# lboss75/vds

Measured on AMD Instinct MI355X. Metric: device-resident encode+repair GiB/s, k=16 m=4 64 MiB stripes, 1/2/4/8 GPU, higher is better.
Workload: dtype u16

## Files before the change

vds_amd/csrc/restore_syn.hpp:

```cpp
#pragma once

#include "ec_device.hpp"

namespace vds_ec {

constexpr int64_t kNoBound = 0x7FFFFFFFFFFFFFFFll;

template <int K, int N, int WV> struct RestorePrograms;

template <int K, int N, int WV>
struct SynShape {
  static constexpr int kWaves = WV;
  static constexpr int kThreads = 64 * WV;
  static constexpr int kM = N - K;
  static constexpr int kLoadPer = K / WV;
  using P = RestorePrograms<K, N, WV>;
  static constexpr int kSynRows = P::kSynRows;
  static constexpr int kCells = P::kIntRows / 16;
  static constexpr int kLdsBytes = N * 16 * 64 * 4;
  static constexpr int kWavesPerSimd = (160 * 1024 / kLdsBytes) * WV / 4;
  static constexpr bool kPrio = 160 * 1024 / kLdsBytes >= 2;
  static_assert(K % WV == 0 && kM <= WV, "survivor loads and erased slots must map onto waves");
  static_assert(kSynRows == 16 && kM == WV, "scatter recovery needs one whole syndrome per wave");
  static_assert(kCells == 2 || kCells == 4, "row split must be b128 / word-group aligned");
// ... 129 lines not shown
      if (first[c])
#pragma unroll
        for (int b = 0; b < 16; ++b) cells[16 * (c0 + c) + b] = 0u;
  }
}

template <int K, int N, int WV, int W>
__device__ __forceinline__ void syn_interp_gm(int wave, const SynLds &L, uint32_t (&cells)[16 * (K / WV)], Stamps &st) {
  static_assert((K == 16 && WV == 4) || (K == 32 && WV == 8),
                "the one-level interpolation is laid out for k = 16 and k = 32");
  using P = RestorePrograms<K, N, WV>;
  constexpr int kPairs = (K / 2) / WV;
  constexpr int kHalfCells = P::kHalfRows / 16;
  constexpr int kParts = WV / 2;
  constexpr bool kPrio = SynShape<K, N, WV>::kPrio;
  if constexpr (W < WV) {
    if (wave != W) return syn_interp_gm<K, N, WV, W + 1>(wave, L, cells, st);
    syn_prio<1, kPrio>();
    syn_gm_stage_a<W, kPairs>(L);
    syn_prio<0, kPrio>();
    st.mark(7);
    __syncthreads();
    st.mark(8);
    uint32_t half[P::kHalfRows];
    P::interpB(W, L, half);
    st.mark(9);
    __syncthreads();
    st.mark(10);
#pragma unroll
    for (int c = 0; c < kHalfCells; ++c) {
      uint32_t v[16];
#pragma unroll
      for (int b = 0; b < 16; ++b) v[b] = half[16 * c + b];
      syn_put_point(L, (K / 2) * (W / kParts) + kHalfCells * (W % kParts) + c, v);
    }
    st.mark(11);
    __syncthreads();
    st.mark(12);
    syn_gm_stage_c<K, W, K / WV>(L, cells);
    st.mark(13);
  }
}

template <int EP>
struct S1In {
  const SynLds &L;
  const Plane16 &own;
  __device__ __forceinline__ u32x4 operator()(int g) const {
    if ((g >> 2) == EP) return u32x4{own.p[4 * (g & 3)], own.p[4 * (g & 3) + 1], own.p[4 * (g & 3) + 2], own.p[4 * (g & 3) + 3]};
    return L(g);
  }
};

#ifndef VDS_GM2
#define VDS_GM2 1
#endif
#ifndef VDS_GM2_PRIO
#define VDS_GM2_PRIO 9
#endif
#ifndef VDS_HALF_PRIO
#define VDS_HALF_PRIO 1
#endif
template <int K, int N, int WV, int W, class Tail, class OwnP = void>
__device__ __forceinline__ void syn_interp_gm2(int wave, const SynLds &L, Stamps &st, Tail &&tail,
                                               const Plane16 *own = nullptr) {
  using P = RestorePrograms<K, N, WV>;
  constexpr bool kPrio = SynShape<K, N, WV>::kPrio;
  constexpr int H = K / 2, kWpf = WV / 4, kWpq = WV / 2;
  if constexpr (W < WV) {
    if (wave != W) return syn_interp_gm2<K, N, WV, W + 1, Tail &, OwnP>(wave, L, st, tail, own);
    uint32_t cells[16 * (K / WV)];
    uint32_t acc[64];
    auto cell = [&](int c) -> uint32_t(&)[16] { return *reinterpret_cast<uint32_t(*)[16]>(acc + 16 * c); };
    syn_prio<1, kPrio && (VDS_GM2_PRIO & 1)>();
    if constexpr (__is_same(OwnP, void))
      P::gm_s1_(W, L, acc);
    else
      P::gm_s1_(W, S1In<OwnP::kPoint[W]>{L, *own}, acc);
#pragma unroll
    for (int c = 0; c < 4; ++c) syn_put_point(L, 4 * W + c, cell(c));
    syn_prio<0, kPrio && (VDS_GM2_PRIO & 1)>();
    st.mark(7);
    __syncthreads();
    st.mark(8);
    syn_prio<1, kPrio && (VDS_GM2_PRIO & 2)>();
    P::gm_s2_(W, L, acc);
    constexpr int f = W / kWpf, c0 = 4 * (W % kWpf);
    if constexpr (kWpf > 1) {
      __syncthreads();
      constexpr int h = W % kWpf;
      static_assert(kWpf == 2 && K / 4 == 8, "plane-split S2 is laid out for k = 32");
#pragma unroll
      for (int c = 0; c < 8; ++c)
#pragma unroll
        for (int g = 0; g < 2; ++g)
          L.put(4 * (4 * c + f) + 2 * h + g,
                u32x4{acc[8 * c + 4 * g], acc[8 * c + 4 * g + 1], acc[8 * c + 4 * g + 2], acc[8 * c + 4 * g + 3]});
    } else {
#pragma unroll
      for (int c = 0; c < 4; ++c) syn_put_point(L, 4 * (c0 + c) + f, cell(c));
    }
    syn_prio<0, kPrio && (VDS_GM2_PRIO & 2)>();
    st.mark(9);
    __syncthreads();
    st.mark(10);
    syn_prio<1, kPrio && (VDS_GM2_PRIO & 4)>();
    P::gm_s3sum_(W, L, acc);
    constexpr int par = W / kWpq, i0 = 4 * (W % kWpq);
#pragma unroll
    for (int c = 0; c < 4; ++c) P::gm_twist(i0 + c, cell(c));
    syn_prio<0, kPrio && (VDS_GM2_PRIO & 4)>();
    __syncthreads();
#pragma unroll
    for (int c = 0; c < 4; ++c) syn_put_point(L, H * par + i0 + c, cell(c));
    st.mark(11);
    __syncthreads();
    st.mark(12);
    syn_prio<1, kPrio && (VDS_GM2_PRIO & 8)>();
    syn_gm_stage_c<K, W, K / WV>(L, cells);
    syn_prio<0, kPrio && (VDS_GM2_PRIO & 8)>();
    st.mark(13);
    tail(cells);
  }
}

#define VDS_RS_C(i) [c##i] "+v"(acc.p[i])
#define VDS_RS_A(i) [a##i] "v"(t.p[i])
#define VDS_RS_B(i) [b##i] "v"(t1.p[i])
#define VDS_RS_LIST(M) M(0), M(1), M(2), M(3), M(4), M(5), M(6), M(7), M(8), M(9), M(10), M(11), M(12), M(13), M(14), M(15)
#define VDS_RS_SEQ(M) M(0) M(1) M(2) M(3) M(4) M(5) M(6) M(7) M(8) M(9) M(10) M(11) M(12) M(13) M(14) M(15)
#define VDS_RS_XA(i) "v_xor_b32 %[c" #i "], %[c" #i "], %[a" #i "]\n"
#define VDS_RS_XB(i) "v_xor_b32 %[c" #i "], %[c" #i "], %[b" #i "]\n"
#define VDS_RS_X3(i) "v_bitop3_b32 %[c" #i "], %[c" #i "], %[a" #i "], %[b" #i "] bitop3:0x96\n"
__device__ __forceinline__ void rec_pair(Plane16 &acc, const Plane16 &t, const Plane16 &t1, uint32_t two) {
// ... 95 lines not shown
    return -1;
  }
  __device__ __forceinline__ u32x4 operator()(int idx) const {
    const int i = slot(idx >> 2), g = idx & 3;
    return u32x4{P[i].p[4 * g], P[i].p[4 * g + 1], P[i].p[4 * g + 2], P[i].p[4 * g + 3]};
  }
};
template <int WV, class FillP, bool REGS, int W>
__device__ __forceinline__ void syn_scatter_fill(int wave, const SynLds &L, const Plane16 (&Ps)[4]) {
  if constexpr (W < WV) {
    if (wave != W) return syn_scatter_fill<WV, FillP, REGS, W + 1>(wave, L, Ps);
#pragma unroll
    for (int q = 0; q < FillP::kParts; ++q) {
      uint32_t acc[16 * FillP::kPart];
      if constexpr (REGS)
        FillP::fill_part(q, W, FillRegIn<FillP, W>{Ps}, acc);
      else
        FillP::fill_part(q, W, L, acc);
#pragma unroll
      for (int m = 0; m < FillP::kPart; ++m)
        if (q * FillP::kPart + m < FillP::kFill)
          lds_xor_point(L, FillP::kPoint[q * FillP::kPart + m < FillP::kFill ? q * FillP::kPart + m : 0],
                        *reinterpret_cast<const Plane16 *>(acc + 16 * m));
    }
  }
}

template <class F, class = void>
struct FillOwn {
  static constexpr bool value = false;
};
template <class F>
struct FillOwn<F, decltype(void(F::kOwn))> {
  static constexpr bool value = F::kOwn;
};
template <class FillP, int W>
struct OwnIn {
  const SynLds &L;
  const Plane16 (&P)[4];
  __device__ __forceinline__ u32x4 operator()(int idx) const {
    const int i = FillRegIn<FillP, W>::slot(idx >> 2), g = idx & 3;
    if (i >= 0) return u32x4{P[i].p[4 * g], P[i].p[4 * g + 1], P[i].p[4 * g + 2], P[i].p[4 * g + 3]};
    return L(idx);
  }
};
template <int WV, class FillP, int W>
__device__ __forceinline__ void syn_own_fill(int wave, const SynLds &L, const Plane16 (&Ps)[4], Plane16 &own) {
  if constexpr (W < WV) {
    if (wave != W) return syn_own_fill<WV, FillP, W + 1>(wave, L, Ps, own);
    FillP::template own<W>(OwnIn<FillP, W>{L, Ps}, own.p);
  }
}

__device__ __forceinline__ u32x4 ld16_guard(const uint8_t *p, int64_t valid) {
  if (valid >= 16) return g_ld<4, u32x4>(p);
  u32x4 v = {0u, 0u, 0u, 0u};
  if (valid > 0) {
#pragma unroll
    for (int i = 0; i < 3; ++i)
      if (4 * i + 4 <= valid) v[i] = *(const gmem<uint32_t> *)(p + 4 * i);
    if (valid & 2) v[valid >> 2] = *(const gmem<uint16_t> *)(p + (valid & ~3));
  }
  return v;
}
__device__ __forceinline__ void st16_guard(uint8_t *p, u32x4 v, int64_t valid) {
  if (valid >= 16) {
    g_st<8>(p, v);
  } else if (valid > 0) {
#pragma unroll
    for (int i = 0; i < 3; ++i)
      if (4 * i + 4 <= valid) *(gmem<uint32_t> *)(p + 4 * i) = v[i];
    const int w = (int)(valid >> 2);
    const uint32_t x = v[w];
    for (int b = 0; b < (int)(valid & 3); ++b) ((gmem<uint8_t> *)p)[4 * w + b] = uint8_t(x >> (8 * b));
  }
}

struct NoFill {
  static constexpr int kFill = -1;
  static constexpr bool kScatter = false;
  static constexpr bool kSmall = false;
  static constexpr bool kPerm = false;
  static constexpr bool kMulti = false;
};
constexpr uint32_t kClsSyn = 0, kClsSmall1 = 1, kClsSmall2 = 2, kClsPerm = 3;
template <int K> struct MultiP {
  static constexpr int kFill = -1;
  static constexpr bool kScatter = false, kSmall = false, kPerm = false, kMulti = true;
};
template <class T> struct TypeTag {
  using type = T;
};
template <int K> struct PermSyn;
template <int K, int MS> struct SmallSyn;
#ifndef VDS_SYN_RT2
#define VDS_SYN_RT2 1
#endif
#ifndef VDS_BATCH_DUAL
#define VDS_BATCH_DUAL 1
#endif
#ifndef VDS_RT2_SPREAD
#define VDS_RT2_SPREAD 1
#endif
template <int K, int N, int WV, bool REGEN, bool BATCH, bool RT = false, class FillP = NoFill>
__device__ __forceinline__ void restore_syn_body(const SynRestoreArgs &a) {
  constexpr bool FILL = FillP::kFill >= 0;
  constexpr bool kScatter = FILL && FillP::kScatter;
  constexpr bool kOwn = FILL && FillOwn<FillP>::value;
  static_assert(!kOwn || (K == 16 && !REGEN && !BATCH && !RT), "the own-group fill is a k = 16 restore form");
  constexpr bool kSmall = FillP::kSmall;
  constexpr bool kPerm = FillP::kPerm;
  constexpr bool kMulti = FillP::kMulti;
  static_assert(!kMulti || (BATCH && !RT), "MULTI is a batch mode");
  static_assert(!kSmall || (BATCH && !RT && !FILL), "SMALL is a batch mode of its own");
  static_assert(!kPerm || (BATCH && REGEN && !RT && !FILL), "PERM is a batch regenerate mode of its own");
  using S = SynShape<K, N, WV>;
  using P = typename S::P;
  constexpr bool kPrio = S::kPrio;
  static_assert(!RT || BATCH, "RT is a batch mode");
  extern __shared__ __attribute__((aligned(16))) uint32_t lds[];
  const int lane = threadIdx.x & 63;
  const int wave = __builtin_amdgcn_readfirstlane(threadIdx.x >> 6);
  const BitMasks bm = bit_masks();
  if constexpr (!kPrio && VDS_HALF_PRIO)
    if (wave >= WV / 2) __builtin_amdgcn_s_setprio(1);
  SynLds L;
  L.base = (lds_char *)lds;
  L.lo = 16u * lane;
  L.hi = 16u * lane + 65536u;
  asm volatile("" : "+v"(L.hi));
  if constexpr (N * 16 > 128) {
    L.hi2 = 16u * lane + 131072u;
    asm volatile("" : "+v"(L.hi2));
  } else {
    L.hi2 = L.hi;
  }
  auto obj_of = [&](uint32_t t) -> uint32_t { return t / a.tiles_per_obj; };
  auto stripe0_of = [&](uint32_t t) -> uint64_t { return (uint64_t)(t % a.tiles_per_obj) * kTileStripes; };
  auto half_obj = [&](uint32_t t, int h) -> const SynBatchObj & { return a.objs[s_ld(&a.tiles[t].obj[h])]; };
  auto half_s0 = [&](uint32_t t, int h) -> uint64_t { return s_ld(&a.tiles[t].stripe0[h]); };

  u32x4 Q[S::kLoadPer][4];
  auto load = [&](uint32_t t) {
    if constexpr (BATCH) {
#pragma unroll
      for (int h = 0; h < 2; ++h) {
        const SynBatchObj &d = half_obj(t, h);
        const uint64_t st0 = half_s0(t, h);
        const int64_t valid = (int64_t)s_ld(&d.chunk_len) - (int64_t)(2 * st0);
        const uint8_t *src[S::kLoadPer];
#pragma unroll
        for (int s = 0; s < S::kLoadPer; ++s) src[s] = s_ld(&d.chunks[wave * S::kLoadPer + s]) + 2 * st0 + 16 * lane;
        if (valid >= 2 * (int64_t)kHalfStripes) {
#pragma unroll
          for (int s = 0; s < S::kLoadPer; ++s)
#pragma unroll
            for (int q = 0; q < 2; ++q) Q[s][2 * h + q] = g_ld<4, u32x4>(src[s] + 1024 * q);
        } else {
#pragma unroll
          for (int s = 0; s < S::kLoadPer; ++s)
#pragma unroll
            for (int q = 0; q < 2; ++q) Q[s][2 * h + q] = ld16_guard(src[s] + 1024 * q, valid - 16 * lane - 1024 * q);
        }
      }
    } else {
      const uint32_t ob = obj_of(t);
      const uint64_t st0 = stripe0_of(t);
#pragma unroll
      for (int s = 0; s < S::kLoadPer; ++s) {
        const uint8_t *src = a.chunks[wave * S::kLoadPer + s] + (uint64_t)ob * a.chunk_stride + 2 * st0 + 16 * lane;
#pragma unroll
        for (int q = 0; q < 4; ++q) Q[s][q] = g_ld<4, u32x4>(src + 1024 * q);
      }
    }
  };
  const TileRange tr = tile_range(a.total_tiles);
  Stamps st;
  st.init();
  auto prefetch = [&](uint32_t t) {
    if (t < tr.end && (VDS_DIAG_LOADS != 2 || t == tr.first)) {
      st.rt((t - tr.first) / tr.step);
      load(VDS_DIAG_LOADS == 1 ? tr.first : t);
    } else {
#pragma unroll
      for (int s = 0; s < S::kLoadPer; ++s)
#pragma unroll
        for (int q = 0; q < 4; ++q) Q[s][q] = u32x4{0u, 0u, 0u, 0u};
    }
  };
  constexpr bool kLateLoad = ((K == 32 || BATCH) && !REGEN) || RT;
  const uint32_t t_step = tr.step;
  prefetch(tr.first);
  if constexpr (!REGEN && !BATCH) {
    if (tr.first < tr.end) {
      const uint32_t t0 = tr.first;
      uint8_t *g0 = a.out + (uint64_t)(t0 / a.tiles_per_obj) * a.out_stride +
                    (uint64_t)(t0 % a.tiles_per_obj) * kTileStripes * (2 * K) + 16384u * wave + 16u * lane;
#pragma unroll
      for (int i = 0; i < 16; ++i) g_st<8>(g0 + 1024 * i, u32x4{0u, 0u, 0u, 0u});
    }
  }
  for (uint32_t tile = tr.first; tile < tr.end; tile += t_step) {
    const uint32_t o = BATCH ? 0u : obj_of(tile);
    const uint64_t stripe0 = BATCH ? 0u : stripe0_of(tile);
    const SynBatchPlan *pl = (BATCH && !RT) ? &a.plans[s_ld(&a.tiles[tile].plan)] : nullptr;
    auto erased_of = [&](int m) -> int { return (int)s_ld_u8(BATCH ? pl->erased : a.erased, m); };
    const uint32_t cls = kMulti ? s_ld(&pl->cls) : (kPerm ? kClsPerm : kClsSyn);
    const bool perm_tile = kPerm || (kMulti && REGEN && cls == kClsPerm);
    const int my_erased = RT ? K + wave : perm_tile ? K : (wave < S::kM ? erased_of(wave) : 0);
    constexpr bool kFillRegs = kScatter && VDS_FILL_REGS && K == 16;
    constexpr bool kKeepPs = RT || kFillRegs || kOwn;
    Plane16 own;
    static_assert(!kKeepPs || S::kLoadPer == 4, "four survivors per wave");
    Plane16 Ps[kKeepPs ? S::kLoadPer : 1];

    constexpr bool kRt2 = VDS_SYN_RT2 && RT && !REGEN && K == 32 && N >= K + 8;
    const bool rt2_tile = kRt2 && s_ld(&a.tiles[tile].mode) == 1u;
    constexpr bool kDual = VDS_BATCH_DUAL && BATCH && !RT && !FILL && !kSmall && !kPerm && K == 32;
    const bool dual_tile = kDual && s_ld(&a.tiles[tile].mode) == kTileDual;
    const SynBatchPlan *pl1 = kDual && dual_tile ? &a.plans[s_ld(&half_obj(tile, 1).plan)] : pl;
    syn_prio<1, kPrio>();
    uint64_t bor[2] = {0, 0};
    {
      if constexpr (kDual) {
        if (dual_tile) {
          static_assert(N % WV == 0, "dual tiles: whole slots per wave");
          const u32x4 z = {0u, 0u, 0u, 0u};
#pragma unroll
          for (int i = 0; i < N / WV; ++i)
#pragma unroll
            for (int g = 0; g < 4; ++g) L.put(4 * ((N / WV) * wave + i) + g, z);
          __syncthreads();
        }
      }
      if (wave < S::kM && (!RT || REGEN) && !FILL && (!perm_tile || wave == 0) && !(kDual && dual_tile)) {
        const u32x4 z = {0u, 0u, 0u, 0u};
#pragma unroll
        for (int g = 0; g < 4; ++g) L.put(4 * my_erased + g, z);
      }
      if constexpr (kScatter) {
        if (wave < FillP::kFill) {
          const u32x4 z = {0u, 0u, 0u, 0u};
#pragma unroll
          for (int g = 0; g < 4; ++g) L.put(4 * (int)FillP::kPoint[wave < FillP::kFill ? wave : 0] + g, z);
        }
      }
      if (rt2_tile) {
        const u32x4 z = {0u, 0u, 0u, 0u};
#pragma unroll
        for (int g = 0; g < 4; ++g) L.put(4 * (K + wave) + g, z);
      }
      if constexpr (RT && !REGEN) {
        bor[0] = s_ld(&half_obj(tile, 0).rt.borrowed);
        bor[1] = s_ld(&half_obj(tile, 1).rt.borrowed);
      }
#pragma unroll
      for (int s = 0; s < S::kLoadPer; ++s) {
        uint32_t W[16];
#pragma unroll
        for (int q = 0; q < 4; ++q)
#pragma unroll
          for (int d = 0; d < 4; ++d) W[4 * q + d] = Q[s][q][d];
        transpose16x2(W, bm);
        uint32_t Pl[16];
#pragma unroll
        for (int b = 0; b < 16; ++b) Pl[b] = W[b ^ 8];
        if constexpr (RT) {
          const int j = wave * S::kLoadPer + s;
#pragma unroll
          for (int b = 0; b < 16; ++b) Ps[s].p[b] = Pl[b];
          if constexpr (!REGEN) {
            const uint32_t keep = (((bor[0] >> j) & 1u) ? 0u : kRtH0) | (((bor[1] >> j) & 1u) ? 0u : kRtH1);
            if (keep != 0xFFFFFFFFu)
#pragma unroll
              for (int b = 0; b < 16; ++b) Pl[b] &= keep;
            syn_put_point(L, j, Pl);
          }
        } else {
          if constexpr (kKeepPs)
#pragma unroll
            for (int b = 0; b < 16; ++b) Ps[s].p[b] = Pl[b];
          const int p0 = (int)s_ld_u8(BATCH ? pl->point : a.point, wave * S::kLoadPer + s);
          const int p1 = kDual && dual_tile ? (int)s_ld_u8(pl1->point, wave * S::kLoadPer + s) : p0;
          if (p0 == p1) {
            syn_put_point(L, p0, Pl);
          } else {
            Plane16 v;
#pragma unroll
            for (int b = 0; b < 16; ++b) v.p[b] = Pl[b] & kRtH0;
            lds_xor_point(L, p0, v);
#pragma unroll
            for (int b = 0; b < 16; ++b) v.p[b] = Pl[b] & kRtH1;
            lds_xor_point(L, p1, v);
          }
        }
      }
    }
    syn_prio<0, kPrio>();
    st.mark(0);
    __syncthreads();
    st.mark(1);
    auto phase_perm = [&](auto tag) {
      using PF = typename decltype(tag)::type;
      const uint32_t tp = (uint32_t)erased_of(0) ^ (uint32_t)K;
      struct PermIn {
        const SynLds &L;
        uint32_t tp;
        __device__ __forceinline__ u32x4 operator()(int g) const { return L(4 * (int)((uint32_t)(g >> 2) ^ tp) + (g & 3)); }
      } in{L, tp};
      uint32_t acc[16];
      PF::part(wave, in, acc);
      lds_xor_point(L, K, *reinterpret_cast<const Plane16 *>(acc));
      if (!kLateLoad) prefetch(tile + t_step);
    };
    auto phase_small = [&](auto tag) {
      using PF = typename decltype(tag)::type;
      const uint32_t nrec = s_ld(&pl->nrec);
      if (nrec != 0) {
        {
          uint32_t acc[16 * PF::kM];
          PF::part(wave, L, acc);
#pragma unroll
          for (int j = 0; j < PF::kM; ++j)
            lds_xor_point(L, PF::kSynSlot + j, *reinterpret_cast<const Plane16 *>(acc + 16 * j));
        }
        st.mark(2);
        __syncthreads();
        st.mark(3);
        constexpr int PW = 16 / WV;
        static_assert(PW == 2 || PW == 4, "plane split: 8 or 4 waves");
        uint32_t sy[PF::kM][16];
#pragma unroll
        for (int j = 0; j < PF::kM; ++j) syn_get_point(L, PF::kSynSlot + j, sy[j]);
#pragma unroll
        for (int m = 0; m < PF::kM; ++m) {
          if ((uint32_t)m >= nrec) break;
          uint32_t o[PW];
#pragma unroll
          for (int i = 0; i < PW; ++i) o[i] = 0u;
#pragma unroll
          for (int j = 0; j < PF::kM; ++j) {
            uint64_t mk;
            if constexpr (PW == 2)
              mk = s_ld(reinterpret_cast<const uint32_t *>(&pl->small_mask[m][j][PW * wave]));
            else
              mk = s_ld(reinterpret_cast<const uint64_t *>(&pl->small_mask[m][j][PW * wave]));
#pragma unroll
            for (int i = 0; i < PW; ++i)
#pragma unroll
              for (int b = 0; b < 16; ++b) o[i] ^= sy[j][b] & (0u - (uint32_t)((mk >> (16 * i + b)) & 1u));
          }
          const int e = (int)s_ld_u8(pl->erased, m);
          lds_char *dst = L.at(4 * e + (PW * wave) / 4) + 4 * ((PW * wave) % 4);
// ... 262 lines not shown
        }
#pragma unroll
        for (int s = 0; s < S::kLoadPer; ++s) {
          uint32_t x[kMC];
#pragma unroll
          for (int m = 0; m < kMC; ++m) x[m] = q0[m][s] | (q1[m][s] << 8);
          __builtin_amdgcn_sched_barrier(0);
          Plane16 tt = Ps[s];
#pragma unroll
          for (int i = 0; i < 16; ++i) asm volatile("" : "+v"(tt.p[i]));
          static_for<0, 8>([&](auto bp) {
            constexpr int b = 2 * decltype(bp)::value;
            __builtin_amdgcn_sched_barrier(0);
            const Plane16 t1 = plane_mulx(tt);
#pragma unroll
            for (int m = 0; m < kMC; ++m) rec_dual_x<b>(ce[m], tt, t1, x[m]);
            if constexpr (b < 14) tt = plane_mulx(t1);
          });
        }
#pragma unroll
        for (int m = 0; m < kMC; ++m) {
          const uint32_t r = m0 + m;
          if (r >= rt_rows) break;
          if constexpr (REGEN) {
            lds_xor_point(L, K + (int)r, ce[m]);
          } else {
            const int p0 = r < ne0 ? (int)s_ld_u8(d0.rt.epoint, (int)r) : -1;
            const int p1 = r < ne1 ? (int)s_ld_u8(d1.rt.epoint, (int)r) : -1;
            if (p0 >= 0 && p0 == p1) {
              lds_xor_point(L, p0, ce[m]);
            } else {
              if (p0 >= 0) {
                Plane16 v;
#pragma unroll
                for (int b = 0; b < 16; ++b) v.p[b] = ce[m].p[b] & vh0;
                lds_xor_point(L, p0, v);
              }
              if (p1 >= 0) {
                Plane16 v;
#pragma unroll
                for (int b = 0; b < 16; ++b) v.p[b] = ce[m].p[b] & vh1;
                lds_xor_point(L, p1, v);
              }
            }
          }
        }
      }
    } else if constexpr (kScatter) {
      if constexpr (kFillRegs)
        syn_scatter_fill<WV, FillP, true, 0>(wave, L, Ps);
      else
        syn_scatter_fill<WV, FillP, false, 0>(wave, L, {});
      if (!kLateLoad) prefetch(tile + t_step);
    } else if constexpr (kOwn) {
      syn_own_fill<WV, FillP, 0>(wave, L, Ps, own);
      if (!kLateLoad) prefetch(tile + t_step);
    } else if constexpr (kPerm) {
      phase_perm(TypeTag<FillP>{});
    } else if constexpr (kSmall) {
      phase_small(TypeTag<FillP>{});
    } else if constexpr (kMulti) {
      if (cls == kClsSmall1) {
        phase_small(TypeTag<SmallSyn<K, 1>>{});
      } else if (cls == kClsSmall2) {
        phase_small(TypeTag<SmallSyn<K, 2>>{});
      } else if (REGEN && cls == kClsPerm) {
        if constexpr (REGEN) phase_perm(TypeTag<PermSyn<K>>{});
      } else {
        phase_syn();
      }
    } else if constexpr (FILL) {
      if (wave < FillP::kFill) {
        uint32_t acc[16];
        FillP::fill(wave, L, acc);
        syn_put_point(L, FillP::kPoint[wave], acc);
      }
      if (!kLateLoad) prefetch(tile + t_step);
    } else {
      phase_syn();
    }
    st.mark(5);
    if constexpr (!kOwn) __syncthreads();
    st.mark(6);
    if constexpr (REGEN) {
      if constexpr (RT) prefetch(tile + t_step);
      if constexpr (BATCH) {
        if (RT ? (uint32_t)wave < rt_rows : perm_tile ? wave == 0 : wave < S::kM) {
          uint32_t Pl[16], W[16];
          syn_get_point(L, my_erased, Pl);
          if constexpr (kDual) {
            const int e1 = dual_tile ? (int)s_ld_u8(pl1->erased, wave) : my_erased;
            if (e1 != my_erased) {
              uint32_t P1[16];
              syn_get_point(L, e1, P1);
#pragma unroll
              for (int b = 0; b < 16; ++b) Pl[b] = __builtin_amdgcn_bitop3_b32(kRtH0, Pl[b], P1[b], 0xCA);
            }
          }
#pragma unroll
          for (int b = 0; b < 16; ++b) W[b ^ 8] = Pl[b];
          transpose16x2(W, bm);
          const uint32_t trailer = s_ld(&a.tiles[tile].trailer);
#pragma unroll
          for (int h = 0; h < 2; ++h) {
            const SynBatchObj &d = half_obj(tile, h);
            uint8_t *const rg = s_ld(&d.regen[wave]);
            if (rg == nullptr) continue;
            const uint64_t st0 = half_s0(tile, h);
            const uint64_t clen = s_ld(&d.chunk_len);
            const int64_t valid = (int64_t)clen - 2 - (int64_t)(2 * st0);
            uint8_t *dst = rg + 2 * st0 + 16 * lane;
            if (valid >= 2 * (int64_t)kHalfStripes) {
#pragma unroll
              for (int q = 0; q < 2; ++q)
                g_st<8>(dst + 1024 * q, u32x4{W[8 * h + 4 * q], W[8 * h + 4 * q + 1], W[8 * h + 4 * q + 2],
                                              W[8 * h + 4 * q + 3]});
            } else {
#pragma unroll
              for (int q = 0; q < 2; ++q)
                st16_guard(dst + 1024 * q,
                           u32x4{W[8 * h + 4 * q], W[8 * h + 4 * q + 1], W[8 * h + 4 * q + 2], W[8 * h + 4 * q + 3]},
                           valid - 16 * lane - 1024 * q);
            }
            if (((trailer >> h) & 1u) && lane == 0)
              *(gmem<uint16_t> *)(rg + clen - 2) = *(const gmem<uint16_t> *)(s_ld(&d.chunks[0]) + clen - 2);
          }
        }
        __syncthreads();
        continue;
      }
      uint8_t *const rg = wave < S::kM ? a.regen[wave] : nullptr;
      if (rg != nullptr) {
        uint32_t Pl[16], W[16];
        syn_get_point(L, my_erased, Pl);
#pragma unroll
        for (int b = 0; b < 16; ++b) W[b ^ 8] = Pl[b];
        transpose16x2(W, bm);
        {
          uint8_t *dst = rg + (uint64_t)o * a.regen_stride + 2 * stripe0 + 16 * lane;
#pragma unroll
          for (int q = 0; q < 4; ++q)
            g_st<8>(dst + 1024 * q, u32x4{W[4 * q], W[4 * q + 1], W[4 * q + 2], W[4 * q + 3]});
        }
      }
      __syncthreads();
      continue;
    }
    {
      constexpr bool kTailInWave = RT || kFillRegs || kOwn;
      auto tail = [&](uint32_t (&cells)[16 * S::kCells]) {
      if (kLateLoad && !BATCH) prefetch(tile + t_step);
      constexpr int kChunks = 4 * K / WV;
      constexpr uint32_t kHalfBytes = kHalfStripes * 2 * K;
      static_assert(kHalfBytes % (1024u * kChunks) == 0, "a wave's copy-out lies in one half");
      struct Target {
        uint8_t *g0;
        int64_t valid;
        bool guard;
      };
      auto target = [&]() -> Target {
        const uint32_t wofs = 1024u * kChunks * wave;
        if constexpr (BATCH) {
          const int h = (int)(wofs / kHalfBytes);
          const SynBatchObj &d = half_obj(tile, h);
          const uint64_t at = half_s0(tile, h) * (2 * K) + (wofs - h * kHalfBytes);
          const int64_t valid = (int64_t)s_ld(&d.out_len) - (int64_t)at;
          return {s_ld(&d.out) + at + 16u * lane, valid, valid < 1024 * kChunks};
        } else {
          return {a.out + (uint64_t)o * a.out_stride + stripe0 * (2 * K) + wofs + 16u * lane,
                  kNoBound, false};
        }
      };
      constexpr int kGroups = S::kCells / 2;
      if constexpr (K == 16) {
        static_assert(S::kCells == 4, "one ds_write_b64 = the wave's 4 cells of a stripe");
        static_assert(2048 * 32 + 256 * 8 <= S::kLdsBytes, "staging layout is for 32-byte stripes");
        syn_prio<2, kPrio>();
        uint32_t rows[2][32];
#pragma unroll
        for (int g = 0; g < kGroups; ++g) {
#pragma unroll
          for (int h = 0; h < 2; ++h)
#pragma unroll
            for (int jb = 0; jb < 16; ++jb) rows[g][16 * h + jb] = cells[16 * (2 * g + h) + (jb ^ 8)];
          transpose32(rows[g], bm);
        }
        __syncthreads();
        st.mark(14);
        lds_char *w0 = L.base + 264u * lane + 8u * wave;
#pragma unroll
        for (int slot = 0; slot < 32; ++slot) {
          const int pi = (slot & 1) ? 16 + (slot >> 1) : (slot >> 1);
          *(__attribute__((address_space(3))) u32x2 *)(w0 + (slot >> 3) * 16896 + (slot & 7) * 32) =
              u32x2{rows[0][pi], rows[1][pi]};
        }
        syn_prio<0, kPrio>();
        st.mark(15);
        if (BATCH) prefetch(tile + t_step);
        __syncthreads();
        st.mark(16);
        const lds_char *r0 = L.base + 1056u * kChunks * wave + 16u * lane + 8u * (lane >> 4);
        const auto [g0, out_valid, guard] = target();
// ... 5 lines not shown
        };
        if (!guard) {
#pragma unroll
          for (int i = 0; i < kChunks; ++i) g_st<8>(g0 + 1024 * i, piece(i));
        } else {
#pragma unroll
          for (int i = 0; i < kChunks; ++i) st16_guard(g0 + 1024 * i, piece(i), out_valid - 16 * lane - 1024 * i);
        }
        st.mark(17);
      } else {
        static_assert(K == 32 && S::kCells == 4 && 2048 * 64 + 256 * 8 <= S::kLdsBytes,
                      "staging layout is for 64-byte stripes");
        __syncthreads();
        st.mark(14);
#pragma unroll
        for (int g = 0; g < 2; ++g) {
          uint32_t rows[32];
#pragma unroll
          for (int h = 0; h < 2; ++h)
#pragma unroll
            for (int jb = 0; jb < 16; ++jb) rows[16 * h + jb] = cells[16 * (2 * g + h) + (jb ^ 8)];
          transpose32(rows, bm);
          lds_char *w0 = L.base + 520u * lane + 4u * (2 * wave + g);
#pragma unroll
          for (int slot = 0; slot < 32; ++slot) {
            const int pi = (slot & 1) ? 16 + (slot >> 1) : (slot >> 1);
            *(__attribute__((address_space(3))) uint32_t *)(w0 + (slot >> 3) * (32768 + 512) + (slot & 7) * 64) =
                rows[pi];
          }
        }
        st.mark(15);
        if (BATCH) prefetch(tile + t_step);
        __syncthreads();
        st.mark(16);
        static_assert(kChunks == 16, "16 KiB of copy-out per wave");
        const lds_char *r0 = L.base + 16640u * wave + 64u * (lane >> 2) + 8u * (lane >> 5) + 16u * (lane & 3);
        const auto [g0, out_valid, guard] = target();
        auto piece = [&](int i) {
          const lds_char *r = r0 + 1040 * i;
          const u32x2 v0 = *(__attribute__((address_space(3))) const u32x2 *)r;
          const u32x2 v1 = *(__attribute__((address_space(3))) const u32x2 *)(r + 8);
          return u32x4{v0[0], v0[1], v1[0], v1[1]};
        };
        if (!guard) {
#pragma unroll
          for (int i = 0; i < 16; ++i) g_st<8>(g0 + 1024 * i, piece(i));
        } else {
#pragma unroll
          for (int i = 0; i < 16; ++i) st16_guard(g0 + 1024 * i, piece(i), out_valid - 16 * lane - 1024 * i);
        }
        st.mark(17);
      }
      };
      if constexpr (VDS_GM2 != 0 && kOwn) {
        syn_interp_gm2<K, N, WV, 0, decltype(tail) &, FillP>(wave, L, st, tail, &own);
      } else if constexpr (VDS_GM2 != 0 && kTailInWave) {
        syn_interp_gm2<K, N, WV, 0>(wave, L, st, tail);
      } else if constexpr (VDS_GM2 != 0) {
        uint32_t cells[16 * S::kCells];
        syn_interp_gm2<K, N, WV, 0>(wave, L, st, [&](uint32_t (&c)[16 * S::kCells]) {
#pragma unroll
          for (int i = 0; i < 16 * S::kCells; ++i) cells[i] = c[i];
        });
        tail(cells);
      } else {
        uint32_t cells[16 * S::kCells];
        syn_interp_gm<K, N, WV, 0>(wave, L, cells, st);
        tail(cells);
      }
    }
    __syncthreads();
    st.mark(18);
  }
  st.flush(blockIdx.x * WV + wave, lane);
}

}
```

vds_amd/csrc/vds_ec_jit.cpp:

```cpp
#include <dlfcn.h>
#include <fcntl.h>
#include <hip/hip_runtime.h>
#include <spawn.h>
#include <sys/stat.h>
#include <sys/wait.h>
#include <unistd.h>

#include <cerrno>

#include <atomic>
#include <condition_variable>
#include <cstdlib>
#include <cstring>
#include <deque>
#include <map>
#include <memory>
#include <mutex>
#include <string>
#include <thread>
#include <tuple>
#include <vector>

#include "ec_internal.hpp"
#include "vds_ec.h"
#include "xorprog.hpp"

extern char **environ;

#ifndef VDS_GM2
#define VDS_GM2 1
#endif
#ifndef VDS_GM2_PRIO
#define VDS_GM2_PRIO 9
#endif
#ifndef VDS_HALF_PRIO
#define VDS_HALF_PRIO 1
#endif
#ifndef VDS_FILL_REGS
#define VDS_FILL_REGS 1
#endif
#ifndef VDS_DIAG_STAMPS
#define VDS_DIAG_STAMPS 0
#endif
#ifndef VDS_EC_ARCH_STR
#define VDS_EC_ARCH_STR "gfx950"
#endif

namespace vds_ec {
namespace {


constexpr int kJitMaxDev = 64;
constexpr size_t kJitMaxEntries = 256;
#ifndef VDS_JIT_PB
#define VDS_JIT_PB 3
#endif
#ifndef VDS_JIT_PREFETCH
#define VDS_JIT_PREFETCH 1
#endif
static_assert(VDS_JIT_PB > 0 && VDS_JIT_PB <= 32, "fill block size");
constexpr int fill_block() { return VDS_JIT_PB; }
constexpr bool fill_prefetch() { return VDS_JIT_PREFETCH != 0; }
#ifndef VDS_JIT_SCATTER
#define VDS_JIT_SCATTER 1
#endif
constexpr bool fill_scatter() { return VDS_JIT_SCATTER != 0; }
#ifndef VDS_JIT_OWN
#define VDS_JIT_OWN 0
#endif

std::atomic<int> &jit_mode_ref() {
  static std::atomic<int> m{[] {
    const char *v = std::getenv("VDS_EC_JIT");
    if (!v) return 1;
    if (!std::strcmp(v, "0") || !std::strcmp(v, "off")) return 0;
    if (!std::strcmp(v, "sync")) return 2;
    return 1;
  }()};
  return m;
}
int jit_mode() { return jit_mode_ref().load(std::memory_order_relaxed); }
constexpr int kJitSightings = 2;
constexpr size_t kJitMaxSeen = 1 << 14;

struct Key {
  uint32_t k, n;
  uint64_t survivors;
  uint32_t regen = 0;
  bool operator<(const Key &o) const {
    return std::tie(k, n, survivors, regen) < std::tie(o.k, o.n, o.survivors, o.regen);
  }
};

struct Entry {
  enum State { kPending, kReady, kFailed };
  State state = kPending;
  std::vector<char> code;
  std::string log;
  std::string cache_file;
  hipModule_t mod[kJitMaxDev] = {};
  std::atomic<hipFunction_t> fn[kJitMaxDev] = {};
};

std::string kernel_name(const Key &key) {
  char b[96];
  std::snprintf(b, sizeof b, "vds_ec_jit_%s_%u_%u_%llx", key.regen ? "regen" : "restore", key.k, key.n,
                (unsigned long long)key.survivors);
  return b;
}

std::string kernel_source(const Key &key) {
  const int K = (int)key.k, N = (int)key.n, WV = K / 4;
  std::vector<int> sp;
  for (int a = 0; a < N; ++a)
    if ((key.survivors >> a) & 1u) sp.push_back(a);
  std::string s;
  xorgen::appendf(s,
                  "#define VDS_GM2 %d\n#define VDS_GM2_PRIO %d\n#define VDS_HALF_PRIO %d\n"
                  "#define VDS_FILL_REGS %d\n",
                  VDS_GM2, VDS_GM2_PRIO, VDS_HALF_PRIO, VDS_FILL_REGS);
#if VDS_DIAG_STAMPS
  xorgen::appendf(s, "#define VDS_DIAG_STAMPS 1\n");
#endif
#if defined(VDS_DIAG_LOADS) && VDS_DIAG_LOADS
  xorgen::appendf(s, "#define VDS_DIAG_LOADS %d\n", VDS_DIAG_LOADS);
#endif
  xorgen::appendf(s, "#define VDS_SCHED_FENCE() __builtin_amdgcn_sched_barrier(0)\n#include \"restore_syn.hpp\"\n");
  xorgen::appendf(s, "namespace vds_ec {\n#include \"generated/restore_%d_%d_w%d.inc\"\n", K, N, WV);
  if (key.regen) {
    std::vector<int> tg;
    for (int a = 0; a < N; ++a)
      if (!((key.survivors >> a) & 1u)) tg.push_back(a);
    xorgen::emit_fill_scatter(s, "JitFill", K, sp, &tg);
  } else if (VDS_JIT_OWN && xorgen::fill_own_eligible(K, sp)) {
    xorgen::emit_fill_own(s, "JitFill", K, sp, fill_block(), fill_prefetch());
  } else if (fill_scatter()) {
    xorgen::emit_fill_scatter(s, "JitFill", K, sp);
  } else {
    xorgen::emit_fill_programs(s, "JitFill", K, sp, fill_block(), fill_prefetch());
  }
  xorgen::appendf(s, "}  // namespace vds_ec\n");
  xorgen::appendf(s,
                  "extern \"C\" __global__ __launch_bounds__((vds_ec::SynShape<%d, %d, %d>::kThreads), "
                  "(vds_ec::SynShape<%d, %d, %d>::kWavesPerSimd))\n"
                  "void %s(vds_ec::SynRestoreArgs a) {\n"
                  "  vds_ec::restore_syn_body<%d, %d, %d, %s, false, false, vds_ec::JitFill>(a);\n}\n",
                  K, N, WV, K, N, WV, kernel_name(key).c_str(), K, N, WV, key.regen ? "true" : "false");
  return s;
}

std::string helper_path() {
  Dl_info info{};
  if (!dladdr(reinterpret_cast<void *>(&helper_path), &info) || !info.dli_fname) return {};
  std::string p = info.dli_fname;
  const size_t slash = p.rfind('/');
  return (slash == std::string::npos ? std::string(".") : p.substr(0, slash)) + "/vds_ec_jitc";
}

std::string read_file(const std::string &path) {
  std::string out;
  if (FILE *f = std::fopen(path.c_str(), "rb")) {
    char buf[65536];
    size_t n;
    while ((n = std::fread(buf, 1, sizeof buf, f)) > 0) out.append(buf, n);
    std::fclose(f);
  }
  return out;
}

std::string cache_dir() {
  static const std::string d = [] {
    const char *v = std::getenv("VDS_EC_JIT_CACHE");
    if (v && !std::strcmp(v, "0")) return std::string();
    std::string dir;
    if (v && *v) {
      dir = v;
    } else if (const char *x = std::getenv("XDG_CACHE_HOME"); x && *x) {
      dir = std::string(x) + "/vds_ec";
    } else if (const char *h = std::getenv("HOME"); h && *h) {
      dir = std::string(h) + "/.cache";
      (void)mkdir(dir.c_str(), 0700);
      dir += "/vds_ec";
    } else {
      return std::string();
    }
    (void)mkdir(dir.c_str(), 0700);
    return access(dir.c_str(), W_OK) == 0 ? dir : std::string();
  }();
// ... 375 lines not shown
```

vds_amd/csrc/xorprog.hpp:

```cpp
#pragma once

#include <algorithm>
#include <cstdarg>
#include <cstdint>
#include <cstdio>
#include <cstdlib>
#include <string>
#include <unordered_map>
#include <unordered_set>
#include <vector>

#include "gf_common.hpp"

namespace xorgen {

struct XorProgram {
  int ninputs = 0;
  std::vector<std::pair<int, int>> temps;
  std::vector<std::vector<int>> rows;
  size_t xor_count() const {
    size_t n = temps.size();
    for (auto &r : rows) n += r.empty() ? 0 : r.size() - 1;
    return n;
  }
// ... 255 lines not shown
  std::vector<int> v(n);
  for (int i = 0; i < n; ++i) v[i] = row0 + i;
  return v;
}

inline size_t emit_fill_programs(std::string &s, const char *name, int K, const std::vector<int> &spoints, int pb,
                                 bool prefetch = true) {
  std::vector<int> EU;
  for (int a = 0; a < K; ++a)
    if (std::find(spoints.begin(), spoints.end(), a) == spoints.end()) EU.push_back(a);
  std::vector<uint32_t> A(EU.size() * K);
  for (size_t m = 0; m < EU.size(); ++m)
    for (int j = 0; j < K; ++j) {
      uint32_t num = 1, den = 1;
      for (int t = 0; t < K; ++t)
        if (t != j) {
          num = vds_ec::gf16_mul(num, (uint32_t)(EU[m] ^ spoints[t]));
          den = vds_ec::gf16_mul(den, (uint32_t)(spoints[j] ^ spoints[t]));
        }
      A[m * K + j] = vds_ec::gf16_mul(num, vds_ec::gf16_inv(den));
    }
  InputMap im;
  im.map = spoints;
  appendf(s, "struct %s {\n  static constexpr int kFill = %zu;\n  static constexpr bool kScatter = false;\n", name,
          EU.size());
  appendf(s, "  static constexpr bool kSmall = false, kPerm = false, kMulti = false;\n");
  appendf(s, "  static constexpr uint8_t kPoint[%zu] = {", EU.empty() ? (size_t)1 : EU.size());
  for (int e : EU) appendf(s, "%d, ", e);
  appendf(s, "};\n");
  const auto rows = all_bitrows(A, (int)EU.size(), K);
  size_t total = 0;
  for (size_t m = 0; m < EU.size(); ++m) {
    char nm[32];
    std::snprintf(nm, sizeof nm, "fill%zu", m);
    total += emit_program(s, nm, rows, K, row_range(16 * (int)m, 16), pb, im, prefetch);
  }
  appendf(s, "  template <typename In>\n  __device__ __forceinline__ static void fill(int w, const In &IN4, uint32_t (&acc)[16]) {\n");
  appendf(s, "    switch (w) {\n");
  for (size_t m = 0; m < EU.size(); ++m) appendf(s, "      case %zu: fill%zu(IN4, acc); break;\n", m, m);
  appendf(s, "      default: break;\n    }\n  }\n};\n");
  return total;
}

constexpr int kScatterPart = 4;
#ifndef VDS_JIT_SPB
#define VDS_JIT_SPB 2
#endif
#ifndef VDS_JIT_SPREFETCH
#define VDS_JIT_SPREFETCH 1
#endif
static_assert(VDS_JIT_SPB >= 1 && VDS_JIT_SPB <= 4, "scatter block size");
constexpr int scatter_block() { return VDS_JIT_SPB; }
inline size_t emit_fill_scatter(std::string &s, const char *name, int K, const std::vector<int> &spoints,
                                const std::vector<int> *targets = nullptr) {
  std::vector<int> EU;
  if (targets) {
    EU = *targets;
  } else {
    for (int a = 0; a < K; ++a)
      if (std::find(spoints.begin(), spoints.end(), a) == spoints.end()) EU.push_back(a);
  }
  const int F = (int)EU.size(), WV = K / 4, parts = (F + kScatterPart - 1) / kScatterPart;
  std::vector<uint32_t> A((size_t)F * K);
  for (int m = 0; m < F; ++m)
    for (int j = 0; j < K; ++j) {
      uint32_t num = 1, den = 1;
      for (int t = 0; t < K; ++t)
        if (t != j) {
          num = vds_ec::gf16_mul(num, (uint32_t)(EU[m] ^ spoints[t]));
          den = vds_ec::gf16_mul(den, (uint32_t)(spoints[j] ^ spoints[t]));
        }
      A[(size_t)m * K + j] = vds_ec::gf16_mul(num, vds_ec::gf16_inv(den));
    }
  const auto rows = all_bitrows(A, F, K);
  appendf(s, "struct %s {\n  static constexpr int kFill = %d;\n  static constexpr bool kScatter = true;\n", name, F);
  appendf(s, "  static constexpr bool kSmall = false, kPerm = false, kMulti = false;\n");
  appendf(s, "  static constexpr int kParts = %d, kPart = %d;\n", parts, kScatterPart);
  appendf(s, "  static constexpr uint8_t kPoint[%d] = {", F ? F : 1);
  for (int e : EU) appendf(s, "%d, ", e);
  appendf(s, "};\n");
  appendf(s, "  static constexpr uint8_t kSurv[%d] = {", K);
  for (int j = 0; j < K; ++j) appendf(s, "%d, ", spoints[j]);
  appendf(s, "};\n");
  size_t total = 0;
  for (int w = 0; w < WV; ++w)
    for (int q = 0; q < parts; ++q) {
      const int m0 = q * kScatterPart, m1 = std::min(F, m0 + kScatterPart);
      std::vector<std::vector<int>> sub;
      for (int r = 16 * m0; r < 16 * m1; ++r) {
        std::vector<int> row;
        for (int x : rows[r])
          if (x >= 64 * w && x < 64 * w + 64) row.push_back(x - 64 * w);
        sub.push_back(row);
      }
      char nm[48];
      std::snprintf(nm, sizeof nm, "fill%d_%d", w, q);
      InputMap im;
      for (int i = 0; i < 4; ++i) im.map.push_back(spoints[4 * w + i]);
      total += emit_program(s, nm, sub, 4, row_range(0, (int)sub.size()), scatter_block(), im,
                            VDS_JIT_SPREFETCH != 0);
    }
  for (int q = 0; q < parts; ++q) {
    appendf(s, "  template <typename In>\n  __device__ __forceinline__ static void fill_part%d(int w, const In &IN4, uint32_t (&acc)[%d]) {\n",
            q, 16 * kScatterPart);
    appendf(s, "    switch (w) {\n");
    for (int w = 0; w < WV; ++w)
      appendf(s, "      case %d: fill%d_%d(IN4, reinterpret_cast<uint32_t(&)[%d]>(acc)); break;\n", w, w, q,
              16 * (std::min(F, q * kScatterPart + kScatterPart) - q * kScatterPart));
    appendf(s, "      default: break;\n    }\n  }\n");
  }
  appendf(s, "  template <typename In>\n  __device__ __forceinline__ static void fill_part(int q, int w, const In &IN4, uint32_t (&acc)[%d]) {\n",
          16 * kScatterPart);
  appendf(s, "    switch (q) {\n");
  for (int q = 0; q < parts; ++q) appendf(s, "      case %d: fill_part%d(w, IN4, acc); break;\n", q, q);
  appendf(s, "      default: break;\n    }\n  }\n};\n");
  return total;
}

inline bool fill_own_eligible(int K, const std::vector<int> &spoints) {
  if (K != 16) return false;
  for (int w = 0; w < K / 4; ++w) {
    int e = 0;
    for (int a = 4 * w; a < 4 * w + 4; ++a) e += std::find(spoints.begin(), spoints.end(), a) == spoints.end();
    if (e != 1) return false;
  }
  return true;
}
inline size_t emit_fill_own(std::string &s, const char *name, int K, const std::vector<int> &spoints, int pb,
                            bool prefetch = true) {
  if (!fill_own_eligible(K, spoints)) return 0;
  std::vector<int> EU;
  for (int a = 0; a < K; ++a)
    if (std::find(spoints.begin(), spoints.end(), a) == spoints.end()) EU.push_back(a);
  const int F = (int)EU.size();
  std::vector<uint32_t> A((size_t)F * K);
  for (int m = 0; m < F; ++m)
    for (int j = 0; j < K; ++j) {
      uint32_t num = 1, den = 1;
      for (int t = 0; t < K; ++t)
        if (t != j) {
          num = vds_ec::gf16_mul(num, (uint32_t)(EU[m] ^ spoints[t]));
          den = vds_ec::gf16_mul(den, (uint32_t)(spoints[j] ^ spoints[t]));
        }
      A[(size_t)m * K + j] = vds_ec::gf16_mul(num, vds_ec::gf16_inv(den));
    }
  InputMap im;
  im.map = spoints;
  appendf(s, "struct %s {\n  static constexpr int kFill = %d;\n  static constexpr bool kScatter = false, kOwn = true;\n",
          name, F);
  appendf(s, "  static constexpr bool kSmall = false, kPerm = false, kMulti = false;\n");
  appendf(s, "  static constexpr uint8_t kPoint[%d] = {", F);
  for (int e : EU) appendf(s, "%d, ", e);
  appendf(s, "};\n  static constexpr uint8_t kSurv[%d] = {", K);
  for (int j = 0; j < K; ++j) appendf(s, "%d, ", spoints[j]);
  appendf(s, "};\n");
  const auto rows = all_bitrows(A, F, K);
  size_t total = 0;
  for (int m = 0; m < F; ++m) {
    char nm[32];
    std::snprintf(nm, sizeof nm, "own%d", m);
    total += emit_program(s, nm, rows, K, row_range(16 * m, 16), pb, im, prefetch);
  }
  appendf(s, "  template <int W, typename In>\n  __device__ __forceinline__ static void own(const In &IN4, uint32_t (&acc)[16]) {\n");
  for (int m = 0; m < F; ++m) appendf(s, "    %sif constexpr (W == %d) own%d(IN4, acc);\n", m ? "else " : "", m, m);
  appendf(s, "  }\n};\n");
  return total;
}

}
```

Baseline: 1224.

## Add inbox fill form that routes erased-point shares via LDS and drops barriers

```diff
diff --git a/vds_amd/csrc/restore_syn.hpp b/vds_amd/csrc/restore_syn.hpp
--- a/vds_amd/csrc/restore_syn.hpp
+++ b/vds_amd/csrc/restore_syn.hpp
@@ -205,6 +205,31 @@
   }
 };
 
+template <class F, class = void>
+struct FillInbox {
+  static constexpr bool value = false;
+  __device__ __forceinline__ static int order(int j) { return j; }
+};
+template <class F>
+struct FillInbox<F, decltype(void(F::kInbox))> {
+  static constexpr bool value = F::kInbox;
+  __device__ __forceinline__ static int order(int j) { return (int)((F::kOrderPack >> (4 * j)) & 15u); }
+};
+template <class FillP, int W>
+struct S1Regs {
+  const Plane16 (&P)[4];
+  const Plane16 &own;
+  __device__ __forceinline__ u32x4 operator()(int g) const {
+    const int pt = g >> 2, q = g & 3;
+    int i = -1;
+#pragma unroll
+    for (int s = 0; s < 4; ++s)
+      if (FillP::kSurv[4 * W + s] == pt) i = s;
+    if (i < 0) return u32x4{own.p[4 * q], own.p[4 * q + 1], own.p[4 * q + 2], own.p[4 * q + 3]};
+    return u32x4{P[i].p[4 * q], P[i].p[4 * q + 1], P[i].p[4 * q + 2], P[i].p[4 * q + 3]};
+  }
+};
+
 #ifndef VDS_GM2
 #define VDS_GM2 1
 #endif
@@ -214,25 +239,27 @@
 #ifndef VDS_HALF_PRIO
 #define VDS_HALF_PRIO 1
 #endif
-template <int K, int N, int WV, int W, class Tail, class OwnP = void>
+template <int K, int N, int WV, int W, class Tail, class OwnP = void, bool S1 = true>
 __device__ __forceinline__ void syn_interp_gm2(int wave, const SynLds &L, Stamps &st, Tail &&tail,
                                                const Plane16 *own = nullptr) {
   using P = RestorePrograms<K, N, WV>;
   constexpr bool kPrio = SynShape<K, N, WV>::kPrio;
   constexpr int H = K / 2, kWpf = WV / 4, kWpq = WV / 2;
   if constexpr (W < WV) {
-    if (wave != W) return syn_interp_gm2<K, N, WV, W + 1, Tail &, OwnP>(wave, L, st, tail, own);
+    if (wave != W) return syn_interp_gm2<K, N, WV, W + 1, Tail &, OwnP, S1>(wave, L, st, tail, own);
     uint32_t cells[16 * (K / WV)];
     uint32_t acc[64];
     auto cell = [&](int c) -> uint32_t(&)[16] { return *reinterpret_cast<uint32_t(*)[16]>(acc + 16 * c); };
-    syn_prio<1, kPrio && (VDS_GM2_PRIO & 1)>();
-    if constexpr (__is_same(OwnP, void))
-      P::gm_s1_(W, L, acc);
-    else
-      P::gm_s1_(W, S1In<OwnP::kPoint[W]>{L, *own}, acc);
-#pragma unroll
-    for (int c = 0; c < 4; ++c) syn_put_point(L, 4 * W + c, cell(c));
-    syn_prio<0, kPrio && (VDS_GM2_PRIO & 1)>();
+    if constexpr (S1) {
+      syn_prio<1, kPrio && (VDS_GM2_PRIO & 1)>();
+      if constexpr (__is_same(OwnP, void))
+        P::gm_s1_(W, L, acc);
+      else
+        P::gm_s1_(W, S1In<OwnP::kPoint[W]>{L, *own}, acc);
+#pragma unroll
+      for (int c = 0; c < 4; ++c) syn_put_point(L, 4 * W + c, cell(c));
+      syn_prio<0, kPrio && (VDS_GM2_PRIO & 1)>();
+    }
     st.mark(7);
     __syncthreads();
     st.mark(8);
@@ -434,6 +461,50 @@
   }
 }
 
+template <int WV, class FillP, int W>
+__device__ __forceinline__ void syn_inbox_fill(int wave, const SynLds &L, const Plane16 (&Ps)[4], Plane16 &own) {
+  if constexpr (W < WV) {
+    if (wave != W) return syn_inbox_fill<WV, FillP, W + 1>(wave, L, Ps, own);
+    static_assert(FillP::kParts <= 1 && FillP::kFill <= WV, "at most one erased point per group");
+    if constexpr (FillP::kFill > 0) {
+      uint32_t acc[16 * FillP::kPart];
+      FillP::fill_part(0, W, FillRegIn<FillP, W>{Ps}, acc);
+#pragma unroll
+      for (int m = 0; m < FillP::kFill; ++m) {
+        const Plane16 &v = *reinterpret_cast<const Plane16 *>(acc + 16 * m);
+        if (m == FillP::kOwnM[W])
+          own = v;
+        else
+          syn_put_point(L, 4 * (FillP::kPoint[m] / 4) + W, v.p);
+      }
+    }
+  }
+}
+
+template <int K, int N, int WV, class FillP, int W>
+__device__ __forceinline__ void syn_inbox_s1(int wave, const SynLds &L, const Plane16 (&Ps)[4], const Plane16 &own) {
+  if constexpr (W < WV) {
+    if (wave != W) return syn_inbox_s1<K, N, WV, FillP, W + 1>(wave, L, Ps, own);
+    constexpr bool kPrio = SynShape<K, N, WV>::kPrio;
+    syn_prio<1, kPrio && (VDS_GM2_PRIO & 1)>();
+    Plane16 mine;
+    if constexpr (FillP::kOwnM[W] >= 0) {
+      static_assert(WV == 4, "three incoming shares");
+      uint32_t in[WV - 1][16];
+#pragma unroll
+      for (int w = 0; w < WV; ++w)
+        if (w != W) syn_get_point(L, 4 * W + w, in[w < W ? w : w - 1]);
+#pragma unroll
+      for (int b = 0; b < 16; ++b) mine.p[b] = xor3(own.p[b], in[0][b], in[1][b]) ^ in[2][b];
+    }
+    uint32_t acc[64];
+    RestorePrograms<K, N, WV>::gm_s1_(W, S1Regs<FillP, W>{Ps, mine}, acc);
+#pragma unroll
+    for (int c = 0; c < 4; ++c) syn_put_point(L, 4 * W + c, *reinterpret_cast<uint32_t(*)[16]>(acc + 16 * c));
+    syn_prio<0, kPrio && (VDS_GM2_PRIO & 1)>();
+  }
+}
+
 __device__ __forceinline__ u32x4 ld16_guard(const uint8_t *p, int64_t valid) {
   if (valid >= 16) return g_ld<4, u32x4>(p);
   u32x4 v = {0u, 0u, 0u, 0u};
@@ -487,9 +558,11 @@
 template <int K, int N, int WV, bool REGEN, bool BATCH, bool RT = false, class FillP = NoFill>
 __device__ __forceinline__ void restore_syn_body(const SynRestoreArgs &a) {
   constexpr bool FILL = FillP::kFill >= 0;
-  constexpr bool kScatter = FILL && FillP::kScatter;
+  constexpr bool kInbox = FILL && FillInbox<FillP>::value;
+  constexpr bool kScatter = FILL && FillP::kScatter && !kInbox;
   constexpr bool kOwn = FILL && FillOwn<FillP>::value;
   static_assert(!kOwn || (K == 16 && !REGEN && !BATCH && !RT), "the own-group fill is a k = 16 restore form");
+  static_assert(!kInbox || (K == 16 && !REGEN && !BATCH && !RT && VDS_GM2 != 0), "the inbox fill is a k = 16 restore form");
   constexpr bool kSmall = FillP::kSmall;
   constexpr bool kPerm = FillP::kPerm;
   constexpr bool kMulti = FillP::kMulti;
@@ -550,7 +623,8 @@
       const uint64_t st0 = stripe0_of(t);
 #pragma unroll
       for (int s = 0; s < S::kLoadPer; ++s) {
-        const uint8_t *src = a.chunks[wave * S::kLoadPer + s] + (uint64_t)ob * a.chunk_stride + 2 * st0 + 16 * lane;
+        const uint8_t *src = a.chunks[FillInbox<FillP>::order(wave * S::kLoadPer + s)] +
+                             (uint64_t)ob * a.chunk_stride + 2 * st0 + 16 * lane;
 #pragma unroll
         for (int q = 0; q < 4; ++q) Q[s][q] = g_ld<4, u32x4>(src + 1024 * q);
       }
@@ -591,7 +665,7 @@
     const bool perm_tile = kPerm || (kMulti && REGEN && cls == kClsPerm);
     const int my_erased = RT ? K + wave : perm_tile ? K : (wave < S::kM ? erased_of(wave) : 0);
     constexpr bool kFillRegs = kScatter && VDS_FILL_REGS && K == 16;
-    constexpr bool kKeepPs = RT || kFillRegs || kOwn;
+    constexpr bool kKeepPs = RT || kFillRegs || kOwn || kInbox;
     Plane16 own;
     static_assert(!kKeepPs || S::kLoadPer == 4, "four survivors per wave");
     Plane16 Ps[kKeepPs ? S::kLoadPer : 1];
@@ -658,6 +732,9 @@
               for (int b = 0; b < 16; ++b) Pl[b] &= keep;
             syn_put_point(L, j, Pl);
           }
+        } else if constexpr (kInbox) {
+#pragma unroll
+          for (int b = 0; b < 16; ++b) Ps[s].p[b] = Pl[b];
         } else {
           if constexpr (kKeepPs)
 #pragma unroll
@@ -677,10 +754,16 @@
           }
         }
       }
+      if constexpr (kInbox) {
+#pragma unroll
+        for (int s = 0; s < S::kLoadPer; ++s)
+#pragma unroll
+          for (int b = 0; b < 16; ++b) asm volatile("" : "+v"(Ps[s].p[b]));
+      }
     }
     syn_prio<0, kPrio>();
     st.mark(0);
-    __syncthreads();
+    if constexpr (!kInbox) __syncthreads();
     st.mark(1);
     auto phase_perm = [&](auto tag) {
       using PF = typename decltype(tag)::type;
@@ -1049,6 +1132,9 @@
       else
         syn_scatter_fill<WV, FillP, false, 0>(wave, L, {});
       if (!kLateLoad) prefetch(tile + t_step);
+    } else if constexpr (kInbox) {
+      syn_inbox_fill<WV, FillP, 0>(wave, L, Ps, own);
+      prefetch(tile + t_step);
     } else if constexpr (kOwn) {
       syn_own_fill<WV, FillP, 0>(wave, L, Ps, own);
       if (!kLateLoad) prefetch(tile + t_step);
@@ -1077,7 +1163,7 @@
       phase_syn();
     }
     st.mark(5);
-    if constexpr (!kOwn) __syncthreads();
+    if constexpr (!kOwn && !(kInbox && FillP::kFill == 0)) __syncthreads();
     st.mark(6);
     if constexpr (REGEN) {
       if constexpr (RT) prefetch(tile + t_step);
@@ -1144,7 +1230,7 @@
       continue;
     }
     {
-      constexpr bool kTailInWave = RT || kFillRegs || kOwn;
+      constexpr bool kTailInWave = RT || kFillRegs || kOwn || kInbox;
       auto tail = [&](uint32_t (&cells)[16 * S::kCells]) {
       if (kLateLoad && !BATCH) prefetch(tile + t_step);
       constexpr int kChunks = 4 * K / WV;
@@ -1256,7 +1342,11 @@
         st.mark(17);
       }
       };
-      if constexpr (VDS_GM2 != 0 && kOwn) {
+      if constexpr (VDS_GM2 != 0 && kInbox) {
+        static_assert(!kLateLoad, "the inbox form issues the next tile's loads after its fill");
+        syn_inbox_s1<K, N, WV, FillP, 0>(wave, L, Ps, own);
+        syn_interp_gm2<K, N, WV, 0, decltype(tail) &, void, false>(wave, L, st, tail);
+      } else if constexpr (VDS_GM2 != 0 && kOwn) {
         syn_interp_gm2<K, N, WV, 0, decltype(tail) &, FillP>(wave, L, st, tail, &own);
       } else if constexpr (VDS_GM2 != 0 && kTailInWave) {
         syn_interp_gm2<K, N, WV, 0>(wave, L, st, tail);
diff --git a/vds_amd/csrc/vds_ec_jit.cpp b/vds_amd/csrc/vds_ec_jit.cpp
--- a/vds_amd/csrc/vds_ec_jit.cpp
+++ b/vds_amd/csrc/vds_ec_jit.cpp
@@ -68,6 +68,17 @@
 #ifndef VDS_JIT_OWN
 #define VDS_JIT_OWN 0
 #endif
+#ifndef VDS_JIT_INBOX
+#define VDS_JIT_INBOX 1
+#endif
+bool fill_inbox() {
+  static const bool on = [] {
+    const char *v = std::getenv("VDS_EC_JIT_INBOX");
+    if (v && (!std::strcmp(v, "0") || !std::strcmp(v, "1"))) return v[0] == '1';
+    return VDS_JIT_INBOX != 0;
+  }();
+  return on;
+}
 
 std::atomic<int> &jit_mode_ref() {
   static std::atomic<int> m{[] {
@@ -134,6 +145,8 @@
     xorgen::emit_fill_scatter(s, "JitFill", K, sp, &tg);
   } else if (VDS_JIT_OWN && xorgen::fill_own_eligible(K, sp)) {
     xorgen::emit_fill_own(s, "JitFill", K, sp, fill_block(), fill_prefetch());
+  } else if (fill_scatter() && fill_inbox() && xorgen::fill_inbox_eligible(K, sp)) {
+    xorgen::emit_fill_inbox(s, "JitFill", K, sp);
   } else if (fill_scatter()) {
     xorgen::emit_fill_scatter(s, "JitFill", K, sp);
   } else {
diff --git a/vds_amd/csrc/xorprog.hpp b/vds_amd/csrc/xorprog.hpp
--- a/vds_amd/csrc/xorprog.hpp
+++ b/vds_amd/csrc/xorprog.hpp
@@ -331,7 +331,7 @@
 static_assert(VDS_JIT_SPB >= 1 && VDS_JIT_SPB <= 4, "scatter block size");
 constexpr int scatter_block() { return VDS_JIT_SPB; }
 inline size_t emit_fill_scatter(std::string &s, const char *name, int K, const std::vector<int> &spoints,
-                                const std::vector<int> *targets = nullptr) {
+                                const std::vector<int> *targets = nullptr, const std::string *extra = nullptr) {
   std::vector<int> EU;
   if (targets) {
     EU = *targets;
@@ -361,6 +361,7 @@
   appendf(s, "  static constexpr uint8_t kSurv[%d] = {", K);
   for (int j = 0; j < K; ++j) appendf(s, "%d, ", spoints[j]);
   appendf(s, "};\n");
+  if (extra) s += *extra;
   size_t total = 0;
   for (int w = 0; w < WV; ++w)
     for (int q = 0; q < parts; ++q) {
@@ -446,4 +447,40 @@
   return total;
 }
 
-}
+inline bool fill_inbox_eligible(int K, const std::vector<int> &spoints) {
+  if (K != 16 || (int)spoints.size() != K) return false;
+  for (int g = 0; g < K / 4; ++g) {
+    int e = 0;
+    for (int a = 4 * g; a < 4 * g + 4; ++a) e += std::find(spoints.begin(), spoints.end(), a) == spoints.end();
+    if (e > 1) return false;
+  }
+  return true;
+}
+inline size_t emit_fill_inbox(std::string &s, const char *name, int K, const std::vector<int> &spoints) {
+  if (!fill_inbox_eligible(K, spoints)) return 0;
+  std::vector<int> sorted = spoints, extras, owned, EU;
+  std::sort(sorted.begin(), sorted.end());
+  for (int p : sorted)
+    if (p >= K) extras.push_back(p);
+  size_t next_extra = 0;
+  std::string extra = "  static constexpr bool kInbox = true;\n  static constexpr int kOwnM[4] = {";
+  for (int g = 0; g < K / 4; ++g) {
+    int have = 0;
+    for (int a = 4 * g; a < 4 * g + 4; ++a)
+      if (std::binary_search(sorted.begin(), sorted.end(), a)) {
+        owned.push_back(a);
+        ++have;
+      } else {
+        EU.push_back(a);
+      }
+    if (have < 4) owned.push_back(extras[next_extra++]);
+    appendf(extra, "%d, ", have < 4 ? (int)EU.size() - 1 : -1);
+  }
+  uint64_t pack = 0;
+  for (int j = 0; j < K; ++j)
+    pack |= (uint64_t)(std::lower_bound(sorted.begin(), sorted.end(), owned[j]) - sorted.begin()) << (4 * j);
+  appendf(extra, "};\n  static constexpr uint64_t kOrderPack = 0x%016llxull;\n", (unsigned long long)pack);
+  return emit_fill_scatter(s, name, K, owned, nullptr, &extra);
+}
+
+}
```

Result: faster. 1252, median of 6 (+2.3%).
